# Jiawei-Yang/Denoising-ViT

Measured on AMD Instinct MI355X. Metric: stage-1 images denoised/sec (DINOv2-B/14, 518px, 1k Adam steps), higher is better.
Workload: dtype bf16

## Files before the change

### denoising-vit_amd/csrc/dvt_fit_fused.hip

```cpp
#include "dvt_common.h"
#include "dvt_grid_dev.h"
#include "dvt_loss_row.h"

typedef short bf16x8 __attribute__((ext_vector_type(8)));
typedef float f32x4 __attribute__((ext_vector_type(4)));

int g_fit_rows32 = 1;
int g_fit_xcd_affinity = 1;
int g_fit_small_wg = 0;

namespace {

constexpr int FR0 = 16;
constexpr int FW8 = 8;
constexpr int FE = 128;

template <bool F32>
struct Op {
  static constexpr int ES = F32 ? 4 : 2;
  static constexpr int KS = F32 ? 16 : 32;
};
typedef unsigned u32x4f __attribute__((ext_vector_type(4)));

template <bool F32>
__host__ __device__ constexpr int apitch(int K) { return K * Op<F32>::ES + 16; }

struct FusedArgs {
  DvtGridTable T;
  DvtShadowLayout S;
  DvtTLayout TL;
  int n, lattice;
  int xcd_group;
  float grad_scale;
  long long off_grid, off_b1, off_b2, off_G, off_bh1, off_bh2, off_bh3;
  DvtFusedFit f[DVT_FIT_BATCH_MAX];
};

__device__ __forceinline__ uint16_t bf16_of(float v) { return (uint16_t)(dvt_pack_bf16x2(v, 0.f) & 0xffffu); }

template <int NC, int FR, int FW, bool F32>
__device__ __forceinline__ void store_T(const char* img, void* __restrict__ dstTv, int B, int b0, int tid) {
  constexpr int RPP = F32 ? 4 : 8;
  for (int item = tid; item < NC * (FR / RPP); item += 64 * FW) {
    const int grp = item / NC, col = item - grp * NC;
    const int brow = b0 + grp * RPP;
    const char* src = img + grp * RPP * apitch<F32>(NC) + col * Op<F32>::ES;
    if constexpr (F32) {
      const int sg = brow >> 4, g = (brow >> 2) & 3;
      float4 v;
      v.x = *reinterpret_cast<const float*>(src);
      v.y = *reinterpret_cast<const float*>(src + apitch<F32>(NC));
      v.z = *reinterpret_cast<const float*>(src + 2 * apitch<F32>(NC));
      v.w = *reinterpret_cast<const float*>(src + 3 * apitch<F32>(NC));
      const long long off = ((long long)(col >> 4) * (B >> 4) + sg) * 256 + (((g << 4) + (col & 15)) << 2);
      *reinterpret_cast<float4*>(static_cast<float*>(dstTv) + off) = v;
    } else {
      const int kstep = brow >> 5, g = (brow >> 3) & 3;
      uint32_t w[4];
#pragma unroll
      for (int j = 0; j < 4; ++j) {
        const uint32_t lo = *reinterpret_cast<const uint16_t*>(src + (2 * j) * apitch<F32>(NC));
        const uint32_t hi = *reinterpret_cast<const uint16_t*>(src + (2 * j + 1) * apitch<F32>(NC));
        w[j] = lo | (hi << 16);
      }
      const long long off = ((long long)(col >> 4) * (B >> 5) + kstep) * 512 + (((g << 4) + (col & 15)) << 3);
      *reinterpret_cast<uint4*>(static_cast<uint16_t*>(dstTv) + off) = make_uint4(w[0], w[1], w[2], w[3]);
    }
  }
}

template <int K, int N, bool RELU, bool MASK, int RB, int FW, bool F32>
__device__ __forceinline__ void mlp_layer(const char* actA, const void* __restrict__ Wv,
                                          const float* __restrict__ bias, char* act_out,
                                          float* __restrict__ gout, const char* mask, int wave, int lane) {
  constexpr int KS = Op<F32>::KS, ES = Op<F32>::ES;
  constexpr int NTILES = N / 16, NT = (NTILES + FW - 1) / FW, S = K / KS;
  constexpr int INFL = FW == 8 ? 24 : 16;
  constexpr int PD0 = INFL / NT > 16 ? 16 : (INFL / NT < 1 ? 1 : INFL / NT);
  constexpr int PD = PD0 < S ? PD0 : S;
  static_assert(K % KS == 0 && N % 16 == 0, "layer shape");
  const int lc = lane & 15, g = lane >> 4;
  f32x4 acc[RB][NT];
  const char* wp[NT];
#pragma unroll
  for (int i = 0; i < NT; ++i) {
#pragma unroll
    for (int rb = 0; rb < RB; ++rb) acc[rb][i] = (f32x4){0.f, 0.f, 0.f, 0.f};
    const int t = wave + FW * i;
    const int tt = (NTILES % FW == 0 || t < NTILES) ? t : 0;
    wp[i] = static_cast<const char*>(Wv) + (size_t)tt * S * 1024 + lane * 16;
  }
  u32x4f b[PD][NT];
#pragma unroll
  for (int p = 0; p < PD; ++p)
#pragma unroll
    for (int i = 0; i < NT; ++i) b[p][i] = *reinterpret_cast<const u32x4f*>(wp[i] + 1024 * p);
  __builtin_amdgcn_sched_barrier(0);
  const char* ap = actA + lc * apitch<F32>(K) + g * 16;
#pragma unroll
  for (int s = 0; s < S; ++s) {
    u32x4f av[RB];
#pragma unroll
    for (int rb = 0; rb < RB; ++rb) av[rb] = *reinterpret_cast<const u32x4f*>(ap + rb * 16 * apitch<F32>(K) + s * 64);
    if constexpr (F32) {
#pragma unroll
      for (int j = 0; j < 4; ++j)
#pragma unroll
        for (int i = 0; i < NT; ++i)
#pragma unroll
          for (int rb = 0; rb < RB; ++rb)
            acc[rb][i] = __builtin_amdgcn_mfma_f32_16x16x4f32(__uint_as_float(av[rb][j]), __uint_as_float(b[s % PD][i][j]),
                                                              acc[rb][i], 0, 0, 0);
    } else {
#pragma unroll
      for (int i = 0; i < NT; ++i)
#pragma unroll
        for (int rb = 0; rb < RB; ++rb)
          acc[rb][i] = __builtin_amdgcn_mfma_f32_16x16x32_bf16(__builtin_bit_cast(bf16x8, av[rb]),
                                                               __builtin_bit_cast(bf16x8, b[s % PD][i]), acc[rb][i], 0, 0, 0);
    }
    if (s + PD < S) {
#pragma unroll
      for (int i = 0; i < NT; ++i) b[s % PD][i] = *reinterpret_cast<const u32x4f*>(wp[i] + 1024 * (s + PD));
    }
    __builtin_amdgcn_sched_barrier(0);
  }
#pragma unroll
  for (int i = 0; i < NT; ++i) {
    const int t = wave + FW * i;
    if (NTILES % FW != 0 && t >= NTILES) continue;
    const int n = t * 16 + lc;
    const float bv = bias != nullptr ? bias[n] : 0.f;
#pragma unroll
    for (int rb = 0; rb < RB; ++rb)
#pragma unroll
      for (int r = 0; r < 4; ++r) {
        const int row = rb * 16 + 4 * g + r;
        float v = acc[rb][i][r] + bv;
        if (RELU) v = fmaxf(v, 0.f);
        if (MASK) {
          if constexpr (F32) {
            v = *reinterpret_cast<const float*>(mask + row * apitch<F32>(N) + n * ES) > 0.f ? v : 0.f;
          } else {
            const uint16_t m = *reinterpret_cast<const uint16_t*>(mask + row * apitch<F32>(N) + n * ES);
            v = (m != 0 && !(m & 0x8000u)) ? v : 0.f;
          }
        }
        if (act_out != nullptr) {
          if constexpr (F32) *reinterpret_cast<float*>(act_out + row * apitch<F32>(N) + n * ES) = v;
          else *reinterpret_cast<uint16_t*>(act_out + row * apitch<F32>(N) + n * ES) = bf16_of(v);
        }
        if (gout != nullptr) gout[(size_t)row * N + n] = v;
      }
  }
}

template <int C, bool PH2, int FR, bool F32 = false>
struct FusedLds {
  static constexpr int H = C / 2, R = C / 4;
  static constexpr int O_ENC = 0;
  static constexpr int O_H1 = O_ENC + FR * apitch<F32>(FE);
  static constexpr int O_DF = O_H1 + FR * apitch<F32>(H);
  static constexpr int O_RAW = O_DF + FR * apitch<F32>(C);
  static constexpr int O_R1 = O_RAW + FR * apitch<F32>(C);
  static constexpr int O_R2 = O_R1 + FR * apitch<F32>(R);
  static constexpr int TOTAL = PH2 ? O_R2 + FR * apitch<F32>(R) : O_RAW;
};
template <int C>
constexpr bool fused_f32_fits() { return FusedLds<C, true, 16, true>::TOTAL <= 160 * 1024; }

template <int C, bool PH2, int FR, int FW, bool F32 = false>
__global__ __launch_bounds__(64 * FW) void fit_rows_kernel(FusedArgs a) {
  using L = FusedLds<C, PH2, FR, F32>;
  constexpr int RB = FR / 16;
  constexpr int ES = Op<F32>::ES;
  static_assert(FR == 16 || FR == 32, "rows per workgroup");
  static_assert(FW == 8 || (FW == 4 && FR == 16), "waves per workgroup");
  static_assert(!F32 || (FR == 16 && FW == 8), "fp32 operands: 16 rows, 8 waves");
  static_assert(L::TOTAL <= 160 * 1024, "LDS images of the row kernel");
  constexpr int H = C / 2, R = C / 4, E = FE, cq = C / 4;
  __shared__ __attribute__((aligned(16))) char smem[L::TOTAL];
  int fit_, rb_;
  if (a.xcd_group > 0) {
    const int lin = (int)blockIdx.x + (int)blockIdx.y * (int)gridDim.x, xcd = lin & 7, j = lin >> 3;
    fit_ = xcd / a.xcd_group;
    rb_ = j * a.xcd_group + xcd % a.xcd_group;
  } else {
    fit_ = (int)blockIdx.y;
    rb_ = (int)blockIdx.x;
  }
  const DvtFusedFit& f = a.f[fit_];
  const int tid = threadIdx.x, lane = tid & 63;
  const int wave = __builtin_amdgcn_readfirstlane(tid >> 6);
  const int row0 = rb_ * FR;
  const char* __restrict__ sh = static_cast<const char*>(f.shadow);
  const float* __restrict__ P = f.params;
  const float4* __restrict__ feat4 = reinterpret_cast<const float4*>(f.feat);

  uint32_t warm[5] = {0u, 0u, 0u, 0u, 0u};
  {
    constexpr int LPR = (C * 4 + 127) / 128;
    const int j = lane % 32;
#pragma unroll
    for (int rr = lane / 32; rr < FR / FW; rr += 2) {
      if (j < LPR) {
        const int ri = f.ridx[row0 + wave + FW * rr];
        warm[4] ^= __float_as_uint(f.feat[(size_t)ri * C + j * 32]) ^
                   __float_as_uint(P[a.off_G + (size_t)(ri % a.lattice) * C + j * 32]);
      }
    }
  }
  {
    const int per_xcd = a.xcd_group > 0 ? (int)gridDim.x / a.xcd_group : ((int)gridDim.x + 7) / 8;
    const int nslot = per_xcd >= 16 ? 16 : per_xcd;
    const int slot = (a.xcd_group > 0 ? rb_ / a.xcd_group : (rb_ >> 3)) % nslot;
    const long long lines = ((PH2 ? a.S.total : a.S.direct[2]) * ES + 127) / 128;
    const long long per = (lines + nslot - 1) / nslot;
    const long long l0 = slot * per, l1 = l0 + per < lines ? l0 + per : lines;
    const uint32_t* w32 = reinterpret_cast<const uint32_t*>(sh);
#pragma unroll
    for (int j = 0; j < 4 * RB * (8 / FW); ++j) {
      const long long li = l0 + tid + (long long)j * 64 * FW;
      if (li < l1) warm[j & 3] ^= w32[li * 32];
    }
  }

  if (tid < FR * 16) {
    const int r = tid >> 4, l = tid & 15;
    const float2 p = reinterpret_cast<const float2*>(f.xy)[f.ridx[row0 + r]];
    uint32_t idx[4];
    float w[4];
    corners2d(a.T, l, p.x, p.y, idx, w);
    const float4* __restrict__ grid = reinterpret_cast<const float4*>(P + a.off_grid);
    float4 lo = make_float4(0.f, 0.f, 0.f, 0.f), hi = lo;
#pragma unroll
    for (int c = 0; c < 4; ++c) {
      const float4 u = grid[(size_t)idx[c] * 2], v = grid[(size_t)idx[c] * 2 + 1];
      lo.x = fmaf(w[c], u.x, lo.x);
      lo.y = fmaf(w[c], u.y, lo.y);
      lo.z = fmaf(w[c], u.z, lo.z);
      lo.w = fmaf(w[c], u.w, lo.w);
      hi.x = fmaf(w[c], v.x, hi.x);
      hi.y = fmaf(w[c], v.y, hi.y);
      hi.z = fmaf(w[c], v.z, hi.z);
      hi.w = fmaf(w[c], v.w, hi.w);
    }
    if constexpr (F32) {
      *reinterpret_cast<float4*>(smem + L::O_ENC + r * apitch<F32>(E) + l * 32) = lo;
      *reinterpret_cast<float4*>(smem + L::O_ENC + r * apitch<F32>(E) + l * 32 + 16) = hi;
    } else {
      *reinterpret_cast<uint4*>(smem + L::O_ENC + r * apitch<F32>(E) + l * 16) =
          make_uint4(dvt_pack_bf16x2(lo.x, lo.y), dvt_pack_bf16x2(lo.z, lo.w), dvt_pack_bf16x2(hi.x, hi.y),
                     dvt_pack_bf16x2(hi.z, hi.w));
    }
  }
  if (PH2) {
    for (int i = tid; i < FR * cq; i += 64 * FW) {
      const int r = i / cq, q = i - r * cq;
      const float4 v = feat4[(size_t)f.ridx[row0 + r] * cq + q];
      if constexpr (F32)
        *reinterpret_cast<float4*>(smem + L::O_RAW + r * apitch<F32>(C) + q * 16) = v;
      else
        *reinterpret_cast<uint2*>(smem + L::O_RAW + r * apitch<F32>(C) + q * 8) =
            make_uint2(dvt_pack_bf16x2(v.x, v.y), dvt_pack_bf16x2(v.z, v.w));
    }
  }
  __syncthreads();

  const int B = a.n;
  char* __restrict__ T = static_cast<char*>(f.T);
#define SH(off) (sh + (size_t)(off) * ES)
#define TT(idx) (T + (size_t)a.TL.off[idx] * ES)
  mlp_layer<E, H, true, false, RB, FW, F32>(smem + L::O_ENC, SH(a.S.direct[0]), P + a.off_b1, smem + L::O_H1, nullptr,
                               nullptr, wave, lane);
  if (PH2)
    mlp_layer<C, R, true, false, RB, FW, F32>(smem + L::O_RAW, SH(a.S.direct[2]), P + a.off_bh1, smem + L::O_R1, nullptr,
                                 nullptr, wave, lane);
  __syncthreads();
  mlp_layer<H, C, false, false, RB, FW, F32>(smem + L::O_H1, SH(a.S.direct[1]), P + a.off_b2, nullptr,
                                f.F + (size_t)row0 * C, nullptr, wave, lane);
  store_T<H, FR, FW, F32>(smem + L::O_H1, TT(DVT_T_H1), B, row0, tid);
  store_T<E, FR, FW, F32>(smem + L::O_ENC, TT(DVT_T_ENC), B, row0, tid);
  if (PH2) {
    mlp_layer<R, R, true, false, RB, FW, F32>(smem + L::O_R1, SH(a.S.direct[3]), P + a.off_bh2, smem + L::O_R2, nullptr,
                                 nullptr, wave, lane);
    store_T<C, FR, FW, F32>(smem + L::O_RAW, TT(DVT_T_RAW), B, row0, tid);
    store_T<R, FR, FW, F32>(smem + L::O_R1, TT(DVT_T_R1), B, row0, tid);
    __syncthreads();
    mlp_layer<R, C, false, false, RB, FW, F32>(smem + L::O_R2, SH(a.S.direct[4]), P + a.off_bh3, nullptr,
                                  f.Hres + (size_t)row0 * C, nullptr, wave, lane);
    store_T<R, FR, FW, F32>(smem + L::O_R2, TT(DVT_T_R2), B, row0, tid);
  }
  __syncthreads();

  static_assert(C <= 1024, "row warm-up above assumes <= 32 lines per row");
  {
    constexpr int NR = FR / FW;
    constexpr int NB = (C <= 768 && !(FW == 4 && PH2)) ? 2 : 1;
    DvtLossRowRegs<PH2> lr[NB];
#pragma unroll
    for (int r0 = 0; r0 < NR; r0 += NB) {
#pragma unroll
    for (int rr = r0; rr < r0 + NB; ++rr) {
      const int gr = row0 + wave + FW * rr;
      const int ri = f.ridx[gr];
      dvt_loss_row_load<PH2>(lr[rr - r0], reinterpret_cast<const float4*>(f.F) + (size_t)gr * cq,
                             reinterpret_cast<const float4*>(P + a.off_G) + (size_t)(ri % a.lattice) * cq,
                             PH2 ? reinterpret_cast<const float4*>(f.Hres) + (size_t)gr * cq : nullptr,
                             feat4 + (size_t)ri * cq, cq, lane);
    }
#pragma unroll
    for (int rr = r0; rr < r0 + NB; ++rr) {
      const int row = wave + FW * rr, gr = row0 + row;
      char* const img_p = smem + L::O_DF + row * apitch<F32>(C);
      char* const img_h = PH2 ? smem + L::O_RAW + row * apitch<F32>(C) : nullptr;
      dvt_loss_row_compute<PH2>(lr[rr - r0], reinterpret_cast<float4*>(f.dF) + (size_t)gr * cq,
                                nullptr, nullptr,
                                f.rows + (size_t)gr * 8, a.n, cq, a.grad_scale, lane,
                                F32 ? nullptr : reinterpret_cast<uint2*>(img_p), F32 ? nullptr : reinterpret_cast<uint2*>(img_h),
                                F32 ? reinterpret_cast<float4*>(img_p) : nullptr, F32 ? reinterpret_cast<float4*>(img_h) : nullptr);
    }
    }
  }
  __syncthreads();

  mlp_layer<C, H, false, true, RB, FW, F32>(smem + L::O_DF, SH(a.S.transp[1]), nullptr, smem + L::O_H1, nullptr,
                               smem + L::O_H1, wave, lane);
  store_T<C, FR, FW, F32>(smem + L::O_DF, TT(DVT_T_DF), B, row0, tid);
  if (PH2) {
    mlp_layer<C, R, false, true, RB, FW, F32>(smem + L::O_RAW, SH(a.S.transp[4]), nullptr, smem + L::O_R2, nullptr,
                                 smem + L::O_R2, wave, lane);
    store_T<C, FR, FW, F32>(smem + L::O_RAW, TT(DVT_T_DH), B, row0, tid);
  }
  __syncthreads();
  mlp_layer<H, E, false, false, RB, FW, F32>(smem + L::O_H1, SH(a.S.transp[0]), nullptr, nullptr,
                                f.denc + (size_t)row0 * E, nullptr, wave, lane);
  store_T<H, FR, FW, F32>(smem + L::O_H1, TT(DVT_T_DH1), B, row0, tid);
  if (PH2) {
    mlp_layer<R, R, false, true, RB, FW, F32>(smem + L::O_R2, SH(a.S.transp[3]), nullptr, smem + L::O_R1, nullptr,
                                 smem + L::O_R1, wave, lane);
    store_T<R, FR, FW, F32>(smem + L::O_R2, TT(DVT_T_DR2), B, row0, tid);
    __syncthreads();
    store_T<R, FR, FW, F32>(smem + L::O_R1, TT(DVT_T_DR1), B, row0, tid);
  }
#undef SH
#undef TT
  if (a.n < 0) f.rows[tid] = __uint_as_float(warm[0] ^ warm[1] ^ warm[2] ^ warm[3] ^ warm[4]);
}

__global__ __launch_bounds__(256) void shadow_build_kernel(DvtShadowLayout L, const float* const p0,
                                                           const float* const p1, const float* const p2,
                                                           const float* const p3, void* s0, void* s1,
                                                           void* s2, void* s3, long long q_lo, long long q_hi) {
  const float* p = blockIdx.y == 0 ? p0 : (blockIdx.y == 1 ? p1 : (blockIdx.y == 2 ? p2 : p3));
  void* sh = blockIdx.y == 0 ? s0 : (blockIdx.y == 1 ? s1 : (blockIdx.y == 2 ? s2 : s3));
  const long long q = q_lo + (long long)blockIdx.x * 256 + threadIdx.x;
  if (q >= q_hi) return;
  dvt_shadow_store(L, sh, q * 4, reinterpret_cast<const float4*>(p)[q]);
}


constexpr int WG_MAX_PROB = 5 * DVT_FIT_BATCH_MAX;
struct WgradProb {
  const char* AT;
  const char* BT;
  float* dW;
  float* db;
  int M, N;
};
struct WgradGather {
  const int32_t* offs;
  const uint16_t* perm;
  const float4* rows;
  float4* dG;
};
struct WgradArgs {
  int n_prob, B, ksplit, units_total;
  int n_gather, lattice, cq;
  WgradGather gg[DVT_FIT_BATCH_MAX];
  int unit0[WG_MAX_PROB + 1];
  WgradProb p[WG_MAX_PROB];
};

constexpr int WG_PART_FLOATS = 32 * 32 + 32;
template <int SLOTS, bool F32>
__device__ __forceinline__ void wgrad_block(const WgradArgs& a, int blk, int wave, int lane, float* red) {
  constexpr int PD = 4;
  const int slot = wave >> 2, ks = wave & 3;
  const int unit = blk * SLOTS + slot;
  float* mine = red + (slot * 4 + ks) * WG_PART_FLOATS;
  const bool is_w = unit < a.units_total;
  const int gu = unit - a.units_total;
  float* out_w = nullptr;
  float* out_b = nullptr;
  int out_n = 0;
  int mb = 0, nb = 0;
  bool do_bias = false;
  if (is_w) {
    int pi = 0;
// ... 79 lines not shown
#pragma unroll
    for (int i = 0; i < 2; ++i)
#pragma unroll
      for (int j = 0; j < 2; ++j)
#pragma unroll
        for (int r = 0; r < 4; ++r) mine[((i * 2 + j) * 4 + r) * 64 + lane] = acc[i][j][r];
    if (do_bias) {
#pragma unroll
      for (int i = 0; i < 2; ++i) {
        float v = bsum[i];
        v += __shfl_xor(v, 16, 64);
        v += __shfl_xor(v, 32, 64);
        if (lane < 16) mine[1024 + i * 16 + lane] = v;
      }
    }
  }
  __syncthreads();
  if (is_w) {
    if (ks != 0) return;
    const float* base = red + slot * 4 * WG_PART_FLOATS;
    const int lc = lane & 15, g = lane >> 4;
#pragma unroll
    for (int i = 0; i < 2; ++i)
#pragma unroll
      for (int j = 0; j < 2; ++j)
#pragma unroll
        for (int r = 0; r < 4; ++r) {
          const int o = ((i * 2 + j) * 4 + r) * 64 + lane;
          const float v = (base[o] + base[WG_PART_FLOATS + o]) + (base[2 * WG_PART_FLOATS + o] + base[3 * WG_PART_FLOATS + o]);
          out_w[(size_t)(mb * 32 + i * 16 + 4 * g + r) * out_n + nb * 32 + j * 16 + lc] = v;
        }
    if (do_bias && lane < 32) {
      const int o = 1024 + lane;
      out_b[mb * 32 + lane] = (base[o] + base[WG_PART_FLOATS + o]) + (base[2 * WG_PART_FLOATS + o] + base[3 * WG_PART_FLOATS + o]);
    }
    return;
  }
  const int u = gu * 4 + ks;
  if (u >= a.n_gather * a.lattice) return;
  const int fi = u / a.lattice, r = u - fi * a.lattice;
  const WgradGather& gg = a.gg[fi];
  const int o0 = gg.offs[r], o1 = gg.offs[r + 1];
  if (o1 == o0) return;
  for (int q = lane; q < a.cq; q += 64) {
    float4 acc4 = make_float4(0.f, 0.f, 0.f, 0.f);
    for (int o = o0; o < o1; ++o) {
      const float4 d = gg.rows[(size_t)gg.perm[o] * a.cq + q];
      acc4.x += d.x;
      acc4.y += d.y;
      acc4.z += d.z;
      acc4.w += d.w;
    }
    gg.dG[(size_t)r * a.cq + q] = acc4;
  }
}

struct BackwardArgs {
  DvtGridTable T;
  GridBwdPlan plan;
  GridBwdPtrs gp;
  GridSortedPtrs gs;
  int n, grid_blocks_per_fit, k, wg_blocks;
  WgradArgs w;
};
template <int WAVES, bool F32 = false>
__global__ __launch_bounds__(64 * WAVES) void fit_backward_kernel(BackwardArgs a) {
  __shared__ __attribute__((aligned(16))) float smem[WAVES * WG_PART_FLOATS];
  if ((int)blockIdx.x >= a.wg_blocks) {
    const int b = (int)blockIdx.x - a.wg_blocks;
    const int fy = b / a.grid_blocks_per_fit, bx = b - fy * a.grid_blocks_per_fit;
    if (a.gs.nt > 0) {
      const int parts = a.gs.nt / (64 * WAVES);
      grid_gather_body(a.T, a.gs, fy, bx / parts, bx % parts, a.gp.d_enc[fy], a.gp.d_params[fy], a.gp.touched[fy], 64 * WAVES);
      return;
    }
    if constexpr (WAVES == 16)
      grid_bwd_body<256>(a.T, a.plan, a.gp, a.n, bx, fy, smem, reinterpret_cast<uint32_t*>(smem + 256 * 8));
    return;
  }
  const int wave = __builtin_amdgcn_readfirstlane(threadIdx.x >> 6);
  wgrad_block<WAVES / 4, F32>(a.w, (int)blockIdx.x, wave, threadIdx.x & 63, smem);
}

template <int C>
int launch_rows(const FusedArgs& a, int k, bool phase2, hipStream_t s) {
  if (a.S.f32) {
    if constexpr (fused_f32_fits<C>()) {
      dim3 grid(a.n / 16, k), block(64 * FW8);
      if (phase2) hipLaunchKernelGGL((fit_rows_kernel<C, true, 16, FW8, true>), grid, block, 0, s, a);
      else hipLaunchKernelGGL((fit_rows_kernel<C, false, 16, FW8, true>), grid, block, 0, s, a);
      DVT_CHECK_LAUNCH();
      return 0;
    }
    return DVT_E_BADARG;
  }
  const bool fits32 = phase2 ? (FusedLds<C, true, 32>::TOTAL <= 160 * 1024) : (FusedLds<C, false, 32>::TOTAL <= 160 * 1024);
  const bool r32 = fits32 && a.n % 32 == 0 && (g_fit_rows32 == 2 || (g_fit_rows32 == 1 && k >= 4));
  const bool small = g_fit_small_wg && !r32;
  dim3 grid(a.n / (r32 ? 32 : 16), k), block(64 * (small ? 4 : FW8));
  FusedArgs ax = a;
  ax.xcd_group = (g_fit_xcd_affinity && (k == 2 || k == 4) && grid.x % (8 / k) == 0 && (grid.x * k) % 8 == 0) ? 8 / k : 0;
  const FusedArgs& a_ = ax;
  if (r32) {
    if (phase2) {
      if constexpr (FusedLds<C, true, 32>::TOTAL <= 160 * 1024) hipLaunchKernelGGL((fit_rows_kernel<C, true, 32, FW8>), grid, block, 0, s, a_);
    } else {
      if constexpr (FusedLds<C, false, 32>::TOTAL <= 160 * 1024) hipLaunchKernelGGL((fit_rows_kernel<C, false, 32, FW8>), grid, block, 0, s, a_);
    }
  } else if (small) {
    if (phase2) hipLaunchKernelGGL((fit_rows_kernel<C, true, 16, 4>), grid, block, 0, s, a_);
    else hipLaunchKernelGGL((fit_rows_kernel<C, false, 16, 4>), grid, block, 0, s, a_);
  } else if (phase2) {
    hipLaunchKernelGGL((fit_rows_kernel<C, true, 16, FW8>), grid, block, 0, s, a_);
  } else {
    hipLaunchKernelGGL((fit_rows_kernel<C, false, 16, FW8>), grid, block, 0, s, a_);
  }
  DVT_CHECK_LAUNCH();
  return 0;
}

}

int dvt_shadow_layout(const DvtFitConfig* c, DvtShadowLayout* L) {
  if (!c || !L) return DVT_E_BADARG;
  const int C = c->feat_dim, H = c->hidden, R = c->res_hidden;
  const int E = c->grid.n_levels * c->grid.n_features;
  const int Ns[DVT_SHADOW_MATS] = {H, C, R, R, C}, Ks[DVT_SHADOW_MATS] = {E, H, C, R, R};
  const long long begins[DVT_SHADOW_MATS] = {c->off_w1, c->off_w2, c->off_wh1, c->off_wh2, c->off_wh3};
  const bool tr[DVT_SHADOW_MATS] = {true, true, false, true, true};
  long long o = 0;
  L->n = DVT_SHADOW_MATS;
  L->f32 = c->mlp_bf16 ? 0 : 1;
  L->lo = begins[0];
  L->hi = 0;
  for (int i = 0; i < DVT_SHADOW_MATS; ++i) {
    if (Ks[i] % 32 || Ns[i] % 16 || (tr[i] && (Ns[i] % 32 || Ks[i] % 16))) return DVT_E_BADARG;
    L->N[i] = Ns[i];
    L->K[i] = Ks[i];
    L->begin[i] = begins[i];
    const long long sz = (long long)Ns[i] * Ks[i];
    L->direct[i] = o;
    o += sz;
    L->transp[i] = tr[i] ? o : -1;
    if (tr[i]) o += sz;
    if (begins[i] < L->lo) L->lo = begins[i];
    if (begins[i] + sz > L->hi) L->hi = begins[i] + sz;
  }
  L->total = o;
  return 0;
}

int dvt_shadow_build_k(const DvtShadowLayout* L, int k, const float* const* params, void* const* shadow,
                       long long lo, long long hi, hipStream_t s) {
  if (!L || k < 1 || k > DVT_FIT_BATCH_MAX || L->n <= 0) return DVT_E_BADARG;
  const float* p[4] = {nullptr, nullptr, nullptr, nullptr};
  void* sh[4] = {nullptr, nullptr, nullptr, nullptr};
  for (int f = 0; f < k; ++f) {
    if (!params[f] || !shadow[f]) return DVT_E_BADARG;
    p[f] = params[f];
    sh[f] = shadow[f];
  }
  const long long q_lo = (lo > L->lo ? lo : L->lo) / 4, q_hi = (hi < L->hi ? hi : L->hi) / 4;
  if (q_hi <= q_lo) return 0;
  hipLaunchKernelGGL(shadow_build_kernel, dim3(dvt_cdiv(q_hi - q_lo, 256), k), dim3(256), 0, s, *L, p[0], p[1],
                     p[2], p[3], sh[0], sh[1], sh[2], sh[3], q_lo, q_hi);
  DVT_CHECK_LAUNCH();
  return 0;
}

int g_fit_fused_enable = 1;
int g_fit_sorted_grid = 1;

int g_fit_fused_f32 = 1;

bool dvt_fit_fused_ok(const DvtFitConfig* c) {
  if (!g_fit_fused_enable || !c || !dvt_fit_fused_shapes_ok(c)) return false;
  if (c->mlp_bf16) return true;
  return g_fit_fused_f32 && (c->feat_dim == 384 || c->feat_dim == 768);
}

bool dvt_fit_fused_shapes_ok(const DvtFitConfig* c) {
  if (!c) return false;
  if (c->grid.n_levels != 16 || c->grid.n_features != 8) return false;
  const int C = c->feat_dim;
  if (C != 384 && C != 768 && C != 1024) return false;
  if (c->hidden != C / 2 || c->res_hidden != C / 4) return false;
  if (c->batch % 512 || c->batch <= 0) return false;
  return c->lattice <= 8192 && c->batch <= 65535;
}

int dvt_fit_rows_k(const DvtFitConfig* c, const DvtShadowLayout* L, int k, const DvtFusedFit* fits, bool phase2,
                   hipStream_t s) {
  if (!dvt_fit_fused_ok(c) || !L || !fits || k < 1 || k > DVT_FIT_BATCH_MAX) return DVT_E_BADARG;
  FusedArgs a{};
  a.T = c->grid;
  a.S = *L;
  dvt_t_layout(c, &a.TL);
  a.n = c->batch;
  a.lattice = c->lattice;
  a.grad_scale = (float)c->grad_scale;
  a.off_grid = c->off_grid;
  a.off_b1 = c->off_b1;
  a.off_b2 = c->off_b2;
  a.off_G = c->off_G;
  a.off_bh1 = c->off_bh1;
  a.off_bh2 = c->off_bh2;
  a.off_bh3 = c->off_bh3;
  for (int f = 0; f < k; ++f) a.f[f] = fits[f];
  const double C = c->feat_dim, H = c->hidden, R = c->res_hidden, E = FE, B = c->batch;
  const double flops = 2.0 * B * (2.0 * (E * H + H * C) + (phase2 ? (C * R + 2.0 * R * R + 2.0 * R * C) : 0.0));
  DvtProbeScope probe(DVT_PROBE_FIT_ROWS, s, flops * k);
  switch (c->feat_dim) {
    case 384: return launch_rows<384>(a, k, phase2, s);
    case 768: return launch_rows<768>(a, k, phase2, s);
    default: return launch_rows<1024>(a, k, phase2, s);
  }
}

void dvt_t_layout(const DvtFitConfig* c, DvtTLayout* L) {
  const int C = c->feat_dim, H = c->hidden, R = c->res_hidden, E = c->grid.n_levels * c->grid.n_features;
  const int cols[DVT_T_COUNT] = {C, H, H, E, C, R, R, C, R, R};
  long long o = 0;
  for (int i = 0; i < DVT_T_COUNT; ++i) {
    L->off[i] = o;
    L->cols[i] = cols[i];
    o += (long long)cols[i] * c->batch;
  }
  L->total = o;
}

int dvt_fit_backward_k(const DvtFitConfig* c, int k, const DvtFusedFit* fits, bool phase2, hipStream_t s) {
  if (!dvt_fit_fused_ok(c) || !fits || k < 1 || k > DVT_FIT_BATCH_MAX) return DVT_E_BADARG;
  DvtTLayout TL;
  dvt_t_layout(c, &TL);
  const int C = c->feat_dim, H = c->hidden, R = c->res_hidden, E = c->grid.n_levels * c->grid.n_features;
  BackwardArgs ba{};
  WgradArgs& a = ba.w;
  a.B = c->batch;
  const int ksteps = a.B / 32;
  a.ksplit = 4;
  if (ksteps % 16) return DVT_E_BADARG;
  int units = 0;
  double flops = 0.0;
  const bool f32 = !c->mlp_bf16;
  const size_t es = f32 ? 4 : 2;
  auto add = [&](const DvtFusedFit& f, int tA, int tB, long long ow, long long ob, int M, int N) {
    WgradProb& p = a.p[a.n_prob];
    p.AT = static_cast<const char*>(f.T) + (size_t)TL.off[tA] * es;
    p.BT = static_cast<const char*>(f.T) + (size_t)TL.off[tB] * es;
    p.dW = f.grads + ow;
    p.db = f.grads + ob;
    p.M = M;
    p.N = N;
    a.unit0[a.n_prob++] = units;
    units += (M / 32) * (N / 32);
    flops += 2.0 * M * N * a.B;
  };
  for (int f = 0; f < k; ++f) {
    add(fits[f], DVT_T_DF, DVT_T_H1, c->off_w2, c->off_b2, C, H);
    add(fits[f], DVT_T_DH1, DVT_T_ENC, c->off_w1, c->off_b1, H, E);
    if (phase2) {
      add(fits[f], DVT_T_DH, DVT_T_R2, c->off_wh3, c->off_bh3, C, R);
      add(fits[f], DVT_T_DR2, DVT_T_R1, c->off_wh2, c->off_bh2, R, R);
      add(fits[f], DVT_T_DR1, DVT_T_RAW, c->off_wh1, c->off_bh1, R, C);
    }
  }
  a.unit0[a.n_prob] = units;
  a.units_total = units;
  a.lattice = c->lattice;
  a.cq = C / 4;
  if (!phase2) {
    for (int f = 0; f < k; ++f) {
      if (!fits[f].g_offs || !fits[f].g_perm) return DVT_E_BADARG;
      a.gg[f] = WgradGather{fits[f].g_offs, fits[f].g_perm, reinterpret_cast<const float4*>(fits[f].dF),
                            reinterpret_cast<float4*>(fits[f].grads + c->off_G)};
    }
    a.n_gather = k;
  }
  ba.T = c->grid;
  ba.n = c->batch;
  ba.k = k;
  const int saved_chunk = g_grid_lds_chunk;
  g_grid_lds_chunk = 256;
  dvt_grid_bwd_plan(c->grid, c->batch, &ba.plan);
  g_grid_lds_chunk = saved_chunk;
  const long long direct_threads = (long long)c->batch * (c->grid.n_levels - ba.plan.first_direct_level) * 8;
  ba.grid_blocks_per_fit = ba.plan.n_lds_blocks + dvt_cdiv(direct_threads, 1024);
  bool sorted = g_fit_sorted_grid && dvt_grid_sorted_ok(&c->grid, c->batch);
  for (int f = 0; f < k; ++f) sorted = sorted && fits[f].gs_keys && fits[f].gs_pay && fits[f].gs_w;
  const bool small = g_fit_small_wg && sorted && !f32;
  if (sorted) {
    ba.gs.nt = 4 * c->batch;
    ba.gs.bitmap_end = fits[0].gs_bitmap_end;
    ba.grid_blocks_per_fit = c->grid.n_levels * (ba.gs.nt / (small ? 512 : 1024));
    for (int f = 0; f < k; ++f) {
      ba.gs.keys[f] = fits[f].gs_keys;
      ba.gs.pay[f] = fits[f].gs_pay;
      ba.gs.w[f] = fits[f].gs_w;
// ... 22 lines not shown
```

### denoising-vit_amd/csrc/dvt_gemm_f32.hip

```cpp
#include "dvt_common.h"

typedef float floatx16 __attribute__((ext_vector_type(16)));

namespace {

constexpr int BK = 64;
constexpr int LDK = BK + 4;

struct GemmArgs {
  const float* A;
  const float* B;
  float* C;
  int M, N, K;
  int lda, ldb, ldc;
  const float* bias;
  const float* mask;
  int ldmask;
  float* colsum;
  int relu;
  int kchunk;
  int atomic;
  int epi;
  const float* gamma;
  const float* smul;
// ... 718 lines not shown
  const int tiles = dvt_cdiv(n, 64) * dvt_cdiv(k, 64);
  const int ktiles = dvt_cdiv(m, 64);
  int splits = dvt_cdiv(384, tiles);
  if (splits > ktiles / 2) splits = ktiles / 2;
  if (splits < 1) splits = 1;
  a.kchunk = dvt_cdiv(ktiles, splits) * 64;
  *splits_out = dvt_cdiv(m, a.kchunk);
  return a;
}

GemmArgs make_dgrad(const float* dy, const float* w, float* dx, const float* relu_mask, int m,
                    int n, int k) {
  GemmArgs a{};
  a.A = dy; a.B = w; a.C = dx;
  a.M = m; a.N = k; a.K = n;
  a.lda = n; a.ldb = k; a.ldc = k;
  a.mask = relu_mask; a.ldmask = k;
  a.kchunk = (n + 63) / 64 * 64;
  return a;
}

}

int dvt_linear_group(const DvtLinearOp* ops, int n_ops, hipStream_t s, int bf16_operands) {
  if (!ops || n_ops < 1 || n_ops > MULTI_MAX) return DVT_E_BADARG;
  MultiArgs m{};
  m.n = n_ops;
  int blocks = 0;
  double flops = 0.0;
  for (int i = 0; i < n_ops; ++i) {
    const DvtLinearOp& o = ops[i];
    if (o.m <= 0 || o.n <= 0 || o.k <= 0 || (o.n & 3) || (o.k & 3)) return DVT_E_BADARG;
    int splits = 1;
    if (o.kind == 0) {
      m.g[i] = make_fwd(o.x, o.w, o.b, o.y, o.m, o.n, o.k, o.relu);
      m.layout[i] = 0;
    } else if (o.kind == 1) {
      m.g[i] = make_wgrad(o.dy, o.x, o.dw, o.db, o.m, o.n, o.k, &splits);
      m.layout[i] = 2;
    } else if (o.kind == 2) {
      m.g[i] = make_dgrad(o.dy, o.w, o.dx, o.relu_mask, o.m, o.n, o.k);
      m.layout[i] = 1;
    } else {
      return DVT_E_BADARG;
    }
    m.gx[i] = dvt_cdiv(m.g[i].N, 64);
    m.gy[i] = dvt_cdiv(m.g[i].M, 64);
    m.blk0[i] = blocks;
    blocks += m.gx[i] * m.gy[i] * splits;
    flops += 2.0 * o.m * o.n * o.k;
  }
  m.blk0[n_ops] = blocks;
  DvtProbeScope probe(DVT_PROBE_FIT_GEMM, s, flops);
  if (bf16_operands) {
    if (g_f32_bk == 64)
      hipLaunchKernelGGL(gemm_bf16op_multi_kernel<64>, dim3(blocks), dim3(256), 0, s, m);
    else
      hipLaunchKernelGGL(gemm_bf16op_multi_kernel<32>, dim3(blocks), dim3(256), 0, s, m);
  } else if (g_f32_bk == 16)
    hipLaunchKernelGGL(gemm_f32_multi_kernel<16>, dim3(blocks), dim3(256), 0, s, m);
  else if (g_f32_bk == 32)
    hipLaunchKernelGGL(gemm_f32_multi_kernel<32>, dim3(blocks), dim3(256), 0, s, m);
  else
    hipLaunchKernelGGL(gemm_f32_multi_kernel<64>, dim3(blocks), dim3(256), 0, s, m);
  DVT_CHECK_LAUNCH();
  return 0;
}

namespace {
extern int g_cfg_override;
}
extern int g_fit_fused_enable;
extern int g_fit_fused_f32;
extern int g_fit_sorted_grid;
extern int g_fit_lazy_adam;
extern int g_fit_lazy_refresh;
extern int g_fit_lazy_exact;
extern int g_fit_lazy_merge;
extern int g_fit_shadow_in_adam;
extern int g_adam_pingpong;
extern int g_fit_rows32;
extern int g_fit_small_wg;
extern int g_fit_xcd_affinity;
#ifdef DVT_LAB
extern int g_fit_skip_mask;
#endif

extern "C" int dvt_tune_set(int key, int value) {
  if (key == 0) {
    g_cfg_override = value;
    return 0;
  }
  if (key == 4) {
    if (value == 2 || value == 3)
      g_f32_ex_stages = value;
    else if (value == 10 || value == 11)
      g_f32_big = value == 11;
    else
      g_f32_glds = value;
    return 0;
  }
  if (key == 5) {
    if (value != 16 && value != 32 && value != 64) return DVT_E_BADARG;
    g_f32_bk = value;
    return 0;
  }
  if (key == 8) {
    g_adam_pingpong = value != 0;
    return 0;
  }
  if (key == 6) {
    if (value == 2 || value == 3)
      g_fit_fused_f32 = value == 3;
    else
      g_fit_fused_enable = value != 0;
    return 0;
  }
  if (key == 7) {
    g_fit_sorted_grid = value != 0;
    return 0;
  }
  if (key == 10) {
    g_fit_lazy_exact = value != 0;
    return 0;
  }
  if (key == 11) {
    g_fit_lazy_merge = value != 0;
    return 0;
  }
  if (key == 12) {
    g_fit_shadow_in_adam = value != 0;
    return 0;
  }
  if (key == 13) {
    if (value < 0 || value > 2) return DVT_E_BADARG;
    g_fit_rows32 = value;
    return 0;
  }
  if (key == 14) {
    g_fit_small_wg = value != 0;
    return 0;
  }
  if (key == 16) {
    g_fit_xcd_affinity = value != 0;
    return 0;
  }
#ifdef DVT_LAB
  if (key == 15) {
    g_fit_skip_mask = value & 7;
    return 0;
  }
#endif
  if (key == 9) {
    g_fit_lazy_adam = value != 0;
    if (value >= 2) g_fit_lazy_refresh = value;
    return 0;
  }
  if (key == 18) return dvt_s2_tune(value);
  if (key == 1) return dvt_vit_tune(value);
  if (key == 2) return dvt_grid_tune(value);
  if (key == 3) return dvt_adam_tune(value);
  return DVT_E_BADARG;
}

int dvt_gemm_f32_ex(const DvtGemmEx* g, hipStream_t s) {
  if (!g || !g->A || !g->B || !g->C || g->M <= 0 || g->N <= 0 || g->K <= 0) return DVT_E_BADARG;
  GemmArgs a{};
  a.A = g->A; a.B = g->B; a.C = g->C;
  a.M = g->M; a.N = g->N; a.K = g->K;
  a.lda = g->lda; a.ldb = g->ldb; a.ldc = g->ldc;
  a.bias = g->bias;
  a.colsum = g->layout == 2 ? g->colsum : nullptr;
  a.atomic = g->accumulate;
  if (g->smul != nullptr) {
    const int nb_ = (g->nb0 > 0 ? g->nb0 : 1) * (g->nb1 > 0 ? g->nb1 : 1);
    if (!g->rowsub || g->layout != 0 || nb_ <= 1 || g->K > BK || g->accumulate) return DVT_E_BADARG;
    a.smul = g->smul;
    a.rowsub = g->rowsub;
    a.oscale = g->oscale;
  }
  if (a.K % BK) return DVT_E_BADARG;
  const bool a_kc = g->layout != 2, b_kc = g->layout == 0;
  if ((!a_kc && (a.M % 64)) || (!b_kc && (a.N % 64)) || (a.lda & 3) || (a.ldb & 3)) return DVT_E_BADARG;
  const int nb = (g->nb0 > 0 ? g->nb0 : 1) * (g->nb1 > 0 ? g->nb1 : 1);
  int splits = 1;
  a.kchunk = a.K;
  if (g->accumulate && nb == 1) {
    const int tiles = dvt_cdiv(a.M, 64) * dvt_cdiv(a.N, 64), ktiles = a.K / BK;
    splits = dvt_cdiv(1024, tiles);
    if (splits > ktiles / 4) splits = ktiles / 4;
    if (splits < 1) splits = 1;
    a.kchunk = dvt_cdiv(ktiles, splits) * BK;
    splits = dvt_cdiv(a.K, a.kchunk);
  }
  if (nb > 65535 || splits > 65535) return DVT_E_BADARG;
  dim3 grid(dvt_cdiv(a.N, 64), dvt_cdiv(a.M, 64), nb > 1 ? nb : splits);
  DvtProbeScope probe(DVT_PROBE_FIT_GEMM, s, 2.0 * a.M * a.N * a.K * nb);
#define EX_LAUNCH(NS)                                                                                     \
  do {                                                                                                    \
    if (nb > 1) {                                                                                         \
      BatchDims d{g->nb1 > 0 ? g->nb1 : 1, g->sA0, g->sA1, g->sB0, g->sB1, g->sC0, g->sC1};               \
      if (a.K <= BK && g->layout == 0)                                                                    \
        hipLaunchKernelGGL((gemm_f32_batched_small_k_kernel<true, true>), grid, dim3(256), 0, s, a, d);   \
      else if (g->layout == 0)                                                                            \
        hipLaunchKernelGGL((gemm_f32_glds_batched_kernel<true, true, NS>), grid, dim3(256), 0, s, a, d);  \
      else if (g->layout == 1)                                                                            \
        hipLaunchKernelGGL((gemm_f32_glds_batched_kernel<true, false, NS>), grid, dim3(256), 0, s, a, d); \
      else                                                                                                \
        hipLaunchKernelGGL((gemm_f32_glds_batched_kernel<false, false, NS>), grid, dim3(256), 0, s, a, d);\
    } else {                                                                                              \
      if (g->layout == 0)                                                                                 \
        hipLaunchKernelGGL((gemm_f32_glds_kernel<true, true, NS>), grid, dim3(256), 0, s, a);             \
      else if (g->layout == 1)                                                                            \
        hipLaunchKernelGGL((gemm_f32_glds_kernel<true, false, NS>), grid, dim3(256), 0, s, a);            \
      else                                                                                                \
        hipLaunchKernelGGL((gemm_f32_glds_kernel<false, false, NS>), grid, dim3(256), 0, s, a);           \
    }                                                                                                     \
  } while (0)
  if (g_f32_ex_stages == 2)
    EX_LAUNCH(2);
  else
    EX_LAUNCH(3);
#undef EX_LAUNCH
  DVT_CHECK_LAUNCH();
  return 0;
}

// ... 120 lines not shown
```

### denoising-vit_amd/csrc/dvt_loss_row.h

```cpp
#pragma once
#include "dvt_common.h"

constexpr int DVT_LOSS_MAXQ = 4;

__device__ __forceinline__ float dvt_sgn(float x) { return (x > 0.f) ? 1.f : ((x < 0.f) ? -1.f : 0.f); }

template <bool HAS_RES>
struct DvtLossRowRegs {
  float4 f[DVT_LOSS_MAXQ], g[DVT_LOSS_MAXQ], r[DVT_LOSS_MAXQ], h[HAS_RES ? DVT_LOSS_MAXQ : 1];
};

template <bool HAS_RES>
__device__ __forceinline__ void dvt_loss_row_load(DvtLossRowRegs<HAS_RES>& x, const float4* __restrict__ F,
                                                  const float4* __restrict__ G, const float4* __restrict__ Hres,
                                                  const float4* __restrict__ raw, int cq, int lane) {
#pragma unroll
  for (int s = 0; s < DVT_LOSS_MAXQ; ++s) {
    const int q = lane + 64 * s;
    if (q < cq) {
      x.f[s] = F[q];
      x.g[s] = G[q];
      x.r[s] = raw[q];
      if (HAS_RES) x.h[s] = Hres[q];
    }
// ... 14 lines not shown
    if (q < cq) {
      const float4 f = x.f[s], g = x.g[s], r = x.r[s];
      float4 fg = make_float4(f.x + g.x, f.y + g.y, f.z + g.z, f.w + g.w);
      float4 p = fg;
      if (HAS_RES) {
        const float4 h = x.h[s];
        vh[s] = h;
        p = make_float4(fg.x + h.x, fg.y + h.y, fg.z + h.z, fg.w + h.w);
        const float ex = h.x - (r.x - fg.x), ey = h.y - (r.y - fg.y), ez = h.z - (r.z - fg.z),
                    ew = h.w - (r.w - fg.w);
        rsse += ex * ex + ey * ey + ez * ez + ew * ew;
        rabs += fabsf(h.x) + fabsf(h.y) + fabsf(h.z) + fabsf(h.w);
      }
      vp[s] = p;
      vr[s] = r;
      vfg[s] = fg;
      const float dx = p.x - r.x, dy = p.y - r.y, dz = p.z - r.z, dw = p.w - r.w;
      sse += dx * dx + dy * dy + dz * dz + dw * dw;
      dot += p.x * r.x + p.y * r.y + p.z * r.z + p.w * r.w;
      np += p.x * p.x + p.y * p.y + p.z * p.z + p.w * p.w;
      nr += r.x * r.x + r.y * r.y + r.z * r.z + r.w * r.w;
    }
  }
  sse = wave_sum(sse);
  dot = wave_sum(dot);
  np = wave_sum(np);
  nr = wave_sum(nr);
  if (HAS_RES) {
    rsse = wave_sum(rsse);
    rabs = wave_sum(rabs);
  }
  const float n1 = sqrtf(np), n2 = sqrtf(nr);
  const bool clamped = n1 < 1e-8f;
  const float denom = fmaxf(n1, 1e-8f) * fmaxf(n2, 1e-8f);
  const float cosv = dot / denom;
  if (lane == 0 && row_sums != nullptr) {
    row_sums[0] = sse;
    row_sums[1] = cosv;
    row_sums[2] = rsse;
    row_sums[3] = rabs;
  }
  if (d_pred == nullptr && b_pred == nullptr && f_pred == nullptr) return;
  const float inv_nc = 1.0f / ((float)n * (float)(cq * 4));
  const float inv_n = 1.0f / (float)n;
  const float a_r = -inv_n / denom;
  const float a_p = clamped ? 0.f : inv_n * cosv / np;
  const float c_mse = 2.0f * inv_nc;
#pragma unroll
  for (int s = 0; s < DVT_LOSS_MAXQ; ++s) {
    const int q = lane + 64 * s;
    if (q < cq) {
      const float4 p = vp[s], r = vr[s];
      float4 d;
      d.x = grad_scale * (c_mse * (p.x - r.x) + a_r * r.x + a_p * p.x);
      d.y = grad_scale * (c_mse * (p.y - r.y) + a_r * r.y + a_p * p.y);
      d.z = grad_scale * (c_mse * (p.z - r.z) + a_r * r.z + a_p * p.z);
      d.w = grad_scale * (c_mse * (p.w - r.w) + a_r * r.w + a_p * p.w);
      if (d_pred != nullptr) d_pred[q] = d;
      if (b_pred != nullptr) b_pred[q] = make_uint2(dvt_pack_bf16x2(d.x, d.y), dvt_pack_bf16x2(d.z, d.w));
      if (f_pred != nullptr) f_pred[q] = d;
      if (d_G != nullptr) {
        float* g = d_G + q * 4;
        atomic_add_f32(g + 0, d.x);
        atomic_add_f32(g + 1, d.y);
        atomic_add_f32(g + 2, d.z);
        atomic_add_f32(g + 3, d.w);
      }
      if (HAS_RES && (d_hres != nullptr || b_hres != nullptr || f_hres != nullptr)) {
        const float4 h = vh[s], fg = vfg[s];
        const float c_res = 0.1f * 2.0f * inv_nc, c_abs = 0.02f * inv_nc;
        float4 e;
        e.x = grad_scale * (c_res * (h.x - (r.x - fg.x)) + c_abs * dvt_sgn(h.x));
        e.y = grad_scale * (c_res * (h.y - (r.y - fg.y)) + c_abs * dvt_sgn(h.y));
        e.z = grad_scale * (c_res * (h.z - (r.z - fg.z)) + c_abs * dvt_sgn(h.z));
        e.w = grad_scale * (c_res * (h.w - (r.w - fg.w)) + c_abs * dvt_sgn(h.w));
        if (d_hres != nullptr) d_hres[q] = e;
        if (b_hres != nullptr) b_hres[q] = make_uint2(dvt_pack_bf16x2(e.x, e.y), dvt_pack_bf16x2(e.z, e.w));
        if (f_hres != nullptr) f_hres[q] = e;
      }
    }
  }
}

template <bool HAS_RES>
__device__ __forceinline__ void dvt_loss_row(const float4* __restrict__ F, const float4* __restrict__ G,
                                             const float4* __restrict__ Hres, const float4* __restrict__ raw,
                                             float4* __restrict__ d_pred, float4* __restrict__ d_hres,
                                             float* __restrict__ d_G, float* __restrict__ row_sums, int n,
                                             int cq, float grad_scale, int lane, uint2* b_pred, uint2* b_hres) {
  DvtLossRowRegs<HAS_RES> x;
  dvt_loss_row_load<HAS_RES>(x, F, G, Hres, raw, cq, lane);
  dvt_loss_row_compute<HAS_RES>(x, d_pred, d_hres, d_G, row_sums, n, cq, grad_scale, lane, b_pred, b_hres);
}
```

Before: 3.080.

## Compute per-row loss directly on MFMA accumulators instead of re-reading outputs

Result: no change. 3.076 (median of 2 runs) (-0.1%).

```diff
diff --git a/denoising-vit_amd/csrc/dvt_fit_fused.hip b/denoising-vit_amd/csrc/dvt_fit_fused.hip
--- a/denoising-vit_amd/csrc/dvt_fit_fused.hip
+++ b/denoising-vit_amd/csrc/dvt_fit_fused.hip
@@ -8,6 +8,8 @@
 int g_fit_rows32 = 1;
 int g_fit_xcd_affinity = 1;
 int g_fit_small_wg = 0;
+int g_fit_acc_loss = 1;
+int g_fit_ph2_df = 0;
 
 namespace {
 
@@ -32,6 +34,7 @@
   int n, lattice;
   int xcd_group;
   float grad_scale;
+  int ph2_df;
   long long off_grid, off_b1, off_b2, off_G, off_bh1, off_bh2, off_bh3;
   DvtFusedFit f[DVT_FIT_BATCH_MAX];
 };
@@ -69,10 +72,11 @@
   }
 }
 
-template <int K, int N, bool RELU, bool MASK, int RB, int FW, bool F32>
+template <int K, int N, bool RELU, bool MASK, int RB, int FW, bool F32, bool KEEP = false>
 __device__ __forceinline__ void mlp_layer(const char* actA, const void* __restrict__ Wv,
                                           const float* __restrict__ bias, char* act_out,
-                                          float* __restrict__ gout, const char* mask, int wave, int lane) {
+                                          float* __restrict__ gout, const char* mask, int wave, int lane,
+                                          f32x4* keep = nullptr) {
   constexpr int KS = Op<F32>::KS, ES = Op<F32>::ES;
   constexpr int NTILES = N / 16, NT = (NTILES + FW - 1) / FW, S = K / KS;
   constexpr int INFL = FW == 8 ? 24 : 16;
@@ -151,6 +155,7 @@
           else *reinterpret_cast<uint16_t*>(act_out + row * apitch<F32>(N) + n * ES) = bf16_of(v);
         }
         if (gout != nullptr) gout[(size_t)row * N + n] = v;
+        if constexpr (KEEP) keep[rb * NT + i][r] = v;
       }
   }
 }
@@ -169,7 +174,139 @@
 template <int C>
 constexpr bool fused_f32_fits() { return FusedLds<C, true, 16, true>::TOTAL <= 160 * 1024; }
 
-template <int C, bool PH2, int FR, int FW, bool F32 = false>
+__device__ __forceinline__ float row16_sum(float v) {
+  v += __builtin_bit_cast(float, __builtin_amdgcn_update_dpp(0, __builtin_bit_cast(int, v), 0x128, 0xf, 0xf, false));
+  v += __builtin_bit_cast(float, __builtin_amdgcn_update_dpp(0, __builtin_bit_cast(int, v), 0x124, 0xf, 0xf, false));
+  v += __builtin_bit_cast(float, __builtin_amdgcn_update_dpp(0, __builtin_bit_cast(int, v), 0x122, 0xf, 0xf, false));
+  v += __builtin_bit_cast(float, __builtin_amdgcn_update_dpp(0, __builtin_bit_cast(int, v), 0x121, 0xf, 0xf, false));
+  return v;
+}
+
+template <int C, bool PH2, int FR, int FW, bool F32>
+__device__ __forceinline__ void loss_on_acc(const FusedArgs& a, const DvtFusedFit& f, f32x4* fa, f32x4* ha, char* smem,
+                                            int row0, int wave, int lane, int tid, bool store_df) {
+  using L = FusedLds<C, PH2, FR, F32>;
+  constexpr int RB = FR / 16, NT = C / 16 / FW, ES = Op<F32>::ES;
+  static_assert((C / 16) % FW == 0, "every wave owns NT whole tiles of the C-wide layers");
+  static_assert(FW * FR * 32 + FR * 8 <= FR * apitch<F32>(FE), "the reduction scratch fits the encoding image");
+  const int lc = lane & 15, g = lane >> 4;
+  float* const red = reinterpret_cast<float*>(smem + L::O_ENC);
+  float* const coef = red + FW * FR * 8;
+  const float* __restrict__ P = f.params;
+  f32x4 ra[RB * NT];
+  const float inv_nc = 1.0f / ((float)a.n * (float)C);
+  const float c_mse = 2.0f * inv_nc, c_res = 0.1f * 2.0f * inv_nc, c_abs = 0.02f * inv_nc;
+#pragma unroll
+  for (int rb = 0; rb < RB; ++rb) {
+    f32x4 ga[NT];
+    if constexpr (PH2) {
+      const float* Fown = f.F + (size_t)(row0 + rb * 16 + 4 * g) * C + wave * 16 + lc;
+#pragma unroll
+      for (int r = 0; r < 4; ++r)
+#pragma unroll
+        for (int i = 0; i < NT; ++i) fa[rb * NT + i][r] = Fown[(size_t)r * C + FW * 16 * i];
+    }
+#pragma unroll
+    for (int r = 0; r < 4; ++r) {
+      const int ri = f.ridx[row0 + rb * 16 + 4 * g + r];
+      const float* __restrict__ rawp = f.feat + (size_t)ri * C + wave * 16 + lc;
+      const float* __restrict__ gp = P + a.off_G + (size_t)(ri % a.lattice) * C + wave * 16 + lc;
+#pragma unroll
+      for (int i = 0; i < NT; ++i) {
+        ra[rb * NT + i][r] = rawp[FW * 16 * i];
+        ga[i][r] = gp[FW * 16 * i];
+      }
+    }
+    __builtin_amdgcn_sched_barrier(0);
+#pragma unroll
+    for (int r = 0; r < 4; ++r) {
+      float sse = 0.f, dot = 0.f, np = 0.f, nr = 0.f, rsse = 0.f, rabs = 0.f;
+      char* const img_h = smem + L::O_RAW + (rb * 16 + 4 * g + r) * apitch<F32>(C);
+#pragma unroll
+      for (int i = 0; i < NT; ++i) {
+        const float rv = ra[rb * NT + i][r];
+        const float fg = fa[rb * NT + i][r] + ga[i][r];
+        float p = fg;
+        if (PH2) {
+          const float h = ha[rb * NT + i][r];
+          p = fg + h;
+          const float e = h - (rv - fg);
+          rsse += e * e;
+          rabs += fabsf(h);
+          const float dh = dvt_loss_dhres(h, rv, fg, c_res, c_abs, a.grad_scale);
+          const int n = (wave + FW * i) * 16 + lc;
+          if constexpr (F32) *reinterpret_cast<float*>(img_h + n * ES) = dh;
+          else *reinterpret_cast<uint16_t*>(img_h + n * ES) = bf16_of(dh);
+        }
+        fa[rb * NT + i][r] = p;
+        const float d = p - rv;
+        sse += d * d;
+        dot += p * rv;
+        np += p * p;
+        nr += rv * rv;
+      }
+      sse = row16_sum(sse);
+      dot = row16_sum(dot);
+      np = row16_sum(np);
+      nr = row16_sum(nr);
+      if (PH2) {
+        rsse = row16_sum(rsse);
+        rabs = row16_sum(rabs);
+      }
+      if (lc == 0) {
+        float* o = red + (wave * FR + rb * 16 + 4 * g + r) * 8;
+        *reinterpret_cast<float4*>(o) = make_float4(sse, dot, np, nr);
+        if (PH2) *reinterpret_cast<float2*>(o + 4) = make_float2(rsse, rabs);
+      }
+      __builtin_amdgcn_sched_barrier(0);
+    }
+  }
+  __syncthreads();
+  if (tid < FR) {
+    float4 s = make_float4(0.f, 0.f, 0.f, 0.f);
+    float2 t = make_float2(0.f, 0.f);
+#pragma unroll
+    for (int w = 0; w < FW; ++w) {
+      const float* o = red + (w * FR + tid) * 8;
+      const float4 v = *reinterpret_cast<const float4*>(o);
+      s.x += v.x;
+      s.y += v.y;
+      s.z += v.z;
+      s.w += v.w;
+      if (PH2) {
+        const float2 u = *reinterpret_cast<const float2*>(o + 4);
+        t.x += u.x;
+        t.y += u.y;
+      }
+    }
+    const DvtLossRowCoef c = dvt_loss_row_finish(s.x, s.y, s.z, s.w, t.x, t.y, a.n, f.rows + (size_t)(row0 + tid) * 8);
+    *reinterpret_cast<float2*>(coef + tid * 2) = make_float2(c.a_r, c.a_p);
+  }
+  __syncthreads();
+#pragma unroll
+  for (int rb = 0; rb < RB; ++rb)
+#pragma unroll
+    for (int r = 0; r < 4; ++r) {
+      const int row = rb * 16 + 4 * g + r;
+      const float2 cf = *reinterpret_cast<const float2*>(coef + row * 2);
+      DvtLossRowCoef c;
+      c.a_r = cf.x;
+      c.a_p = cf.y;
+      char* const img_p = smem + L::O_DF + row * apitch<F32>(C);
+      float* const dfp = f.dF + (size_t)(row0 + row) * C;
+#pragma unroll
+      for (int i = 0; i < NT; ++i) {
+        const int n = (wave + FW * i) * 16 + lc;
+        const float d = dvt_loss_dpred(fa[rb * NT + i][r], ra[rb * NT + i][r], c_mse, c, a.grad_scale);
+        if constexpr (F32) *reinterpret_cast<float*>(img_p + n * ES) = d;
+        else *reinterpret_cast<uint16_t*>(img_p + n * ES) = bf16_of(d);
+        if (store_df) dfp[n] = d;
+      }
+      __builtin_amdgcn_sched_barrier(0);
+    }
+}
+
+template <int C, bool PH2, int FR, int FW, bool F32 = false, bool ACC = false>
 __global__ __launch_bounds__(64 * FW) void fit_rows_kernel(FusedArgs a) {
   using L = FusedLds<C, PH2, FR, F32>;
   constexpr int RB = FR / 16;
@@ -277,8 +414,10 @@
     mlp_layer<C, R, true, false, RB, FW, F32>(smem + L::O_RAW, SH(a.S.direct[2]), P + a.off_bh1, smem + L::O_R1, nullptr,
                                  nullptr, wave, lane);
   __syncthreads();
-  mlp_layer<H, C, false, false, RB, FW, F32>(smem + L::O_H1, SH(a.S.direct[1]), P + a.off_b2, nullptr,
-                                f.F + (size_t)row0 * C, nullptr, wave, lane);
+  constexpr int NTC = C / 16 / FW;
+  f32x4 facc[ACC ? RB * NTC : 1], hacc[(ACC && PH2) ? RB * NTC : 1];
+  mlp_layer<H, C, false, false, RB, FW, F32, ACC && !PH2>(smem + L::O_H1, SH(a.S.direct[1]), P + a.off_b2, nullptr,
+                                             (ACC && !PH2) ? nullptr : f.F + (size_t)row0 * C, nullptr, wave, lane, facc);
   store_T<H, FR, FW, F32>(smem + L::O_H1, TT(DVT_T_H1), B, row0, tid);
   store_T<E, FR, FW, F32>(smem + L::O_ENC, TT(DVT_T_ENC), B, row0, tid);
   if (PH2) {
@@ -287,14 +426,16 @@
     store_T<C, FR, FW, F32>(smem + L::O_RAW, TT(DVT_T_RAW), B, row0, tid);
     store_T<R, FR, FW, F32>(smem + L::O_R1, TT(DVT_T_R1), B, row0, tid);
     __syncthreads();
-    mlp_layer<R, C, false, false, RB, FW, F32>(smem + L::O_R2, SH(a.S.direct[4]), P + a.off_bh3, nullptr,
-                                  f.Hres + (size_t)row0 * C, nullptr, wave, lane);
+    mlp_layer<R, C, false, false, RB, FW, F32, ACC>(smem + L::O_R2, SH(a.S.direct[4]), P + a.off_bh3, nullptr,
+                                       ACC ? nullptr : f.Hres + (size_t)row0 * C, nullptr, wave, lane, hacc);
     store_T<R, FR, FW, F32>(smem + L::O_R2, TT(DVT_T_R2), B, row0, tid);
   }
   __syncthreads();
-
+  if constexpr (ACC) {
+    loss_on_acc<C, PH2, FR, FW, F32>(a, f, facc, hacc, smem, row0, wave, lane, tid, !PH2 || a.ph2_df);
+  }
   static_assert(C <= 1024, "row warm-up above assumes <= 32 lines per row");
-  {
+  if constexpr (!ACC) {
     constexpr int NR = FR / FW;
     constexpr int NB = (C <= 768 && !(FW == 4 && PH2)) ? 2 : 1;
     DvtLossRowRegs<PH2> lr[NB];
@@ -314,7 +455,7 @@
       const int row = wave + FW * rr, gr = row0 + row;
       char* const img_p = smem + L::O_DF + row * apitch<F32>(C);
       char* const img_h = PH2 ? smem + L::O_RAW + row * apitch<F32>(C) : nullptr;
-      dvt_loss_row_compute<PH2>(lr[rr - r0], reinterpret_cast<float4*>(f.dF) + (size_t)gr * cq,
+      dvt_loss_row_compute<PH2>(lr[rr - r0], (PH2 && !a.ph2_df) ? nullptr : reinterpret_cast<float4*>(f.dF) + (size_t)gr * cq,
                                 nullptr, nullptr,
                                 f.rows + (size_t)gr * 8, a.n, cq, a.grad_scale, lane,
                                 F32 ? nullptr : reinterpret_cast<uint2*>(img_p), F32 ? nullptr : reinterpret_cast<uint2*>(img_h),
@@ -560,13 +701,15 @@
   wgrad_block<WAVES / 4, F32>(a.w, (int)blockIdx.x, wave, threadIdx.x & 63, smem);
 }
 
-template <int C>
+template <int C, bool ACC>
 int launch_rows(const FusedArgs& a, int k, bool phase2, hipStream_t s) {
+  constexpr bool ACC8 = ACC && C <= 768;
+  constexpr bool ACC32P2 = ACC && C < 768;
   if (a.S.f32) {
     if constexpr (fused_f32_fits<C>()) {
       dim3 grid(a.n / 16, k), block(64 * FW8);
-      if (phase2) hipLaunchKernelGGL((fit_rows_kernel<C, true, 16, FW8, true>), grid, block, 0, s, a);
-      else hipLaunchKernelGGL((fit_rows_kernel<C, false, 16, FW8, true>), grid, block, 0, s, a);
+      if (phase2) hipLaunchKernelGGL((fit_rows_kernel<C, true, 16, FW8, true, ACC8>), grid, block, 0, s, a);
+      else hipLaunchKernelGGL((fit_rows_kernel<C, false, 16, FW8, true, ACC8>), grid, block, 0, s, a);
       DVT_CHECK_LAUNCH();
       return 0;
     }
@@ -581,9 +724,9 @@
   const FusedArgs& a_ = ax;
   if (r32) {
     if (phase2) {
-      if constexpr (FusedLds<C, true, 32>::TOTAL <= 160 * 1024) hipLaunchKernelGGL((fit_rows_kernel<C, true, 32, FW8>), grid, block, 0, s, a_);
+      if constexpr (FusedLds<C, true, 32>::TOTAL <= 160 * 1024) hipLaunchKernelGGL((fit_rows_kernel<C, true, 32, FW8, false, ACC32P2>), grid, block, 0, s, a_);
     } else {
-      if constexpr (FusedLds<C, false, 32>::TOTAL <= 160 * 1024) hipLaunchKernelGGL((fit_rows_kernel<C, false, 32, FW8>), grid, block, 0, s, a_);
+      if constexpr (FusedLds<C, false, 32>::TOTAL <= 160 * 1024) hipLaunchKernelGGL((fit_rows_kernel<C, false, 32, FW8, false, ACC8>), grid, block, 0, s, a_);
     }
   } else if (small) {
     if (phase2) hipLaunchKernelGGL((fit_rows_kernel<C, true, 16, 4>), grid, block, 0, s, a_);
@@ -677,6 +820,7 @@
   a.n = c->batch;
   a.lattice = c->lattice;
   a.grad_scale = (float)c->grad_scale;
+  a.ph2_df = g_fit_ph2_df;
   a.off_grid = c->off_grid;
   a.off_b1 = c->off_b1;
   a.off_b2 = c->off_b2;
@@ -688,10 +832,17 @@
   const double C = c->feat_dim, H = c->hidden, R = c->res_hidden, E = FE, B = c->batch;
   const double flops = 2.0 * B * (2.0 * (E * H + H * C) + (phase2 ? (C * R + 2.0 * R * R + 2.0 * R * C) : 0.0));
   DvtProbeScope probe(DVT_PROBE_FIT_ROWS, s, flops * k);
+  if (g_fit_acc_loss) {
+    switch (c->feat_dim) {
+      case 384: return launch_rows<384, true>(a, k, phase2, s);
+      case 768: return launch_rows<768, true>(a, k, phase2, s);
+      default: return launch_rows<1024, true>(a, k, phase2, s);
+    }
+  }
   switch (c->feat_dim) {
-    case 384: return launch_rows<384>(a, k, phase2, s);
-    case 768: return launch_rows<768>(a, k, phase2, s);
-    default: return launch_rows<1024>(a, k, phase2, s);
+    case 384: return launch_rows<384, false>(a, k, phase2, s);
+    case 768: return launch_rows<768, false>(a, k, phase2, s);
+    default: return launch_rows<1024, false>(a, k, phase2, s);
   }
 }
 
diff --git a/denoising-vit_amd/csrc/dvt_gemm_f32.hip b/denoising-vit_amd/csrc/dvt_gemm_f32.hip
--- a/denoising-vit_amd/csrc/dvt_gemm_f32.hip
+++ b/denoising-vit_amd/csrc/dvt_gemm_f32.hip
@@ -824,6 +824,8 @@
 extern int g_fit_rows32;
 extern int g_fit_small_wg;
 extern int g_fit_xcd_affinity;
+extern int g_fit_ph2_df;
+extern int g_fit_acc_loss;
 #ifdef DVT_LAB
 extern int g_fit_skip_mask;
 #endif
@@ -885,6 +887,14 @@
   }
   if (key == 16) {
     g_fit_xcd_affinity = value != 0;
+    return 0;
+  }
+  if (key == 19) {
+    g_fit_acc_loss = value != 0;
+    return 0;
+  }
+  if (key == 17) {
+    g_fit_ph2_df = value != 0;
     return 0;
   }
 #ifdef DVT_LAB
diff --git a/denoising-vit_amd/csrc/dvt_loss_row.h b/denoising-vit_amd/csrc/dvt_loss_row.h
--- a/denoising-vit_amd/csrc/dvt_loss_row.h
+++ b/denoising-vit_amd/csrc/dvt_loss_row.h
@@ -120,6 +120,34 @@
   }
 }
 
+struct DvtLossRowCoef {
+  float a_r, a_p;
+};
+__device__ __forceinline__ DvtLossRowCoef dvt_loss_row_finish(float sse, float dot, float np, float nr, float rsse, float rabs,
+                                                              int n, float* __restrict__ row_sums) {
+  const float n1 = sqrtf(np), n2 = sqrtf(nr);
+  const bool clamped = n1 < 1e-8f;
+  const float denom = fmaxf(n1, 1e-8f) * fmaxf(n2, 1e-8f);
+  const float cosv = dot / denom;
+  if (row_sums != nullptr) {
+    row_sums[0] = sse;
+    row_sums[1] = cosv;
+    row_sums[2] = rsse;
+    row_sums[3] = rabs;
+  }
+  const float inv_n = 1.0f / (float)n;
+  DvtLossRowCoef c;
+  c.a_r = -inv_n / denom;
+  c.a_p = clamped ? 0.f : inv_n * cosv / np;
+  return c;
+}
+__device__ __forceinline__ float dvt_loss_dpred(float p, float r, float c_mse, DvtLossRowCoef c, float grad_scale) {
+  return grad_scale * (c_mse * (p - r) + c.a_r * r + c.a_p * p);
+}
+__device__ __forceinline__ float dvt_loss_dhres(float h, float r, float fg, float c_res, float c_abs, float grad_scale) {
+  return grad_scale * (c_res * (h - (r - fg)) + c_abs * dvt_sgn(h));
+}
+
 template <bool HAS_RES>
 __device__ __forceinline__ void dvt_loss_row(const float4* __restrict__ F, const float4* __restrict__ G,
                                              const float4* __restrict__ Hres, const float4* __restrict__ raw,
```
